# zraorg/ZRA

Measured on AMD Instinct MI355X. Metric: compress + RA-decompress GiB/s, 16 GiB @ 64 KiB frames, 1/2/4/8 MI355X, higher is better.
Workload: dtype u8

## Files before the change

zra_amd/csrc/zra_decode.hip:

```cpp
#include "zra_dev.h"
#include "zra_kernels.h"

using namespace zra_dev;

namespace {

constexpr int DEC_THREADS = 64;
constexpr int BATCH = 64;
#ifndef ZRA_XWIN
#define ZRA_XWIN 4032
#endif
constexpr u32 XPRE = 64, XWIN = ZRA_XWIN;
constexpr u32 BLOCK_MAX = 128u << 10;

__constant__ u32 c_ll_base[36] = {0,1,2,3,4,5,6,7,8,9,10,11,12,13,14,15,16,18,20,22,24,28,32,40,48,64,128,256,512,1024,2048,4096,8192,16384,32768,65536};
__constant__ u8 c_ll_bits[36] = {0,0,0,0,0,0,0,0,0,0,0,0,0,0,0,0,1,1,1,1,2,2,3,3,4,6,7,8,9,10,11,12,13,14,15,16};
__constant__ u32 c_ml_base[53] = {3,4,5,6,7,8,9,10,11,12,13,14,15,16,17,18,19,20,21,22,23,24,25,26,27,28,29,30,31,32,33,34,
                                  35,37,39,41,43,47,51,59,67,83,99,131,259,515,1027,2051,4099,8195,16387,32771,65539};
__constant__ u8 c_ml_bits[53] = {0,0,0,0,0,0,0,0,0,0,0,0,0,0,0,0,0,0,0,0,0,0,0,0,0,0,0,0,0,0,0,0,
                                 1,1,1,1,2,2,3,3,4,4,5,7,8,9,10,11,12,13,14,15,16};
__constant__ short c_ll_defnorm[36] = {4,3,2,2,2,2,2,2,2,2,2,2,2,1,1,1,2,2,2,2,2,2,2,2,2,3,2,1,1,1,1,1,-1,-1,-1,-1};
__constant__ short c_ml_defnorm[53] = {1,4,3,2,2,2,2,2,2,1,1,1,1,1,1,1,1,1,1,1,1,1,1,1,1,1,1,1,1,1,1,1,
                                       1,1,1,1,1,1,1,1,1,1,1,1,1,1,-1,-1,-1,-1,-1,-1,-1};
__constant__ short c_of_defnorm[29] = {1,1,1,1,1,1,2,2,2,1,1,1,1,1,1,1,1,1,1,1,1,1,1,1,-1,-1,-1,-1,-1};
__constant__ u16 c_huf_t0[16][2] = {{0,0},{0,0},{38,130},{448,128},{556,128},{714,128},{883,128},{897,128},{926,128},{947,128},{1107,128},{1177,128},{1242,128},{1349,128},{1455,128},{722,128}};
__constant__ u16 c_huf_t1[16][2] = {{1,1},{1,1},{1313,74},{1353,74},{1353,74},{1418,74},{1437,74},{1515,75},{1613,75},{1729,77},{2083,81},{2379,87},{2415,93},{2644,106},{2422,124},{1891,145}};

__device__ __forceinline__ u64 mk_seqsym(u32 baseValue, u32 addBits, u32 nbBits, u32 nextBase) {
  return (u64)baseValue | ((u64)addBits << 32) | ((u64)nbBits << 40) | ((u64)nextBase << 48);
}
__device__ __forceinline__ u32 mk_cell(u32 sym, u32 addBits, u32 nbBits, u32 nextBase) {
  return sym | (addBits << 8) | (nbBits << 16) | (nextBase << 20);
}

// ... 693 lines not shown
      {
        const u32 at = bpos + S.seqPos;
        const u32 got = stage(S.w1, at);
        (void)got;
        wsync();
      }
      const u8* const sw = S.w1 - S.seqPos;
      const u8* const swLim = S.w1 + STAGE_BYTES + 8;
      if (lane == 0) {
        parse_seq_header(S, sw + S.seqPos, bsize - S.seqPos);
        if (S.err) { S.lateErr = S.err; S.err = 0; S.nbSeq = 0; S.seqTables = 0; }
        if (S.alloc && S.nbSeq) {
          const u64 take = ((u64)S.nbSeq + 3) & ~3ull;
          const u64 at = atomicAdd((unsigned long long*)&a.counters[ZRA_DC_SEQCUR], (unsigned long long)take);
          if (at + take > a.seqCap) S.alloc = 0;
          S.seqBase = at;
        }
      }
      wsync();
      if (ALL && (!S.alloc || nBlk >= a.bpf)) { bail = true; break; }
      if (!S.alloc) {
        if (lane == 0) {
          save_persistent(S.hdrPos, produced0, hv0, hmb0, hns0, hx20);
          if (!FUSED) a.nextActive[atomicAdd(&a.counters[ZRA_DC_NNEXT], 1u)] = j;
        }
        handed = true; outcome = 2;
        wsync();
        break;
      }

      PPROF(10)
      const u32 nbSeq = S.nbSeq, regen = S.litRegen;
      const size_t jb = ALL ? (size_t)j * a.bpf + nBlk : (size_t)j;
      u32* const T = ALL ? a.blkTables + jb * ZRA_DEC_TBL_WORDS : a.tables + (size_t)j * ZRA_DEC_TBL_WORDS;
      if (S.seqTables) {
        for (int kind = 0; kind < 3; kind++) {
          const int k = kind == 0 ? 0 : kind == 1 ? 2 : 1;
          const u32 mode = k == 0 ? (S.seqModes >> 6) : k == 2 ? ((S.seqModes >> 4) & 3) : ((S.seqModes >> 2) & 3);
          if (lane == 0) {
            u32 tl = 0, ms = 0, used = 0;
            seq_table_parse(S, k, mode, sw + S.seqPos, bsize - S.seqPos, &tl, &ms, &used, swLim);
            S.seqPos += used; S.tl = tl; S.ms = ms;
            if (mode == 3) { u32 v = k == 0 ? S.llValid : k == 1 ? S.mlValid : S.ofValid; if (!v) S.err = ZE_CORRUPTION; }
            if (S.err) { S.lateErr = S.err; S.err = 0; }
          }
          wsync();
          PPROF(11)
          if (S.lateErr) break;
          const u32 tl = S.tl, ms = S.ms;
          u32* const G = T + (k == 0 ? ZRA_DEC_TBL_LL : k == 1 ? ZRA_DEC_TBL_ML : ZRA_DEC_TBL_OF);
          if (mode == 1) {
            if (lane == 0) {
              if (k == 2) { G[0] = mk_cell(ms, ms, 0, 0); S.ofShare = (ms > 22) ? 256u : 0u; }
              else G[0] = mk_cell(ms, k == 0 ? c_ll_bits[ms] : c_ml_bits[ms], 0, 0);
              if (FUSED) { u32* const GL = ldsT + (k == 0 ? ZRA_LDS_TBL_LL : k == 1 ? ZRA_LDS_TBL_ML : ZRA_LDS_TBL_OF); GL[0] = G[0]; if (k != 2) GL[1] = k == 0 ? c_ll_base[ms] : c_ml_base[ms]; }
            }
          } else if (mode != 3) {
            build_fse_dtable(S.stage, S.norm, ms, tl, k, S.spread, (u64*)S.w0, S.wnext, lane);
            wsync();
            const u32 words = (k == 2 ? 1u : 2u) << tl;
            if (!FUSED) for (u32 i = lane; i < (1u << tl); i += DEC_THREADS) G[i] = S.stage[k == 2 ? i : 2 * i];
            if (FUSED) { u32* const GL = ldsT + (k == 0 ? ZRA_LDS_TBL_LL : k == 1 ? ZRA_LDS_TBL_ML : ZRA_LDS_TBL_OF); for (u32 i = lane; i < words; i += DEC_THREADS) GL[i] = S.stage[i]; }
            if (k == 2) {
              u32 cnt = 0;
              for (u32 i = lane; i < (1u << tl); i += DEC_THREADS) cnt += (S.stage[i] & 0xFF) > 22;
              cnt = wave_sum(cnt);
              if (lane == 0) S.ofShare = cnt << (8 - tl);
            }
            wsync();
          }
          if (lane == 0 && mode != 3) {
            if (k == 0) { S.llLog = tl; S.llValid = 1; } else if (k == 1) { S.mlLog = tl; S.mlValid = 1; } else { S.ofLog = tl; S.ofValid = 1; }
          }
          if (ALL) {
            if (mode == 3 && prevT[k] && prevT[k] != G) {
              const u32 lg = k == 0 ? S.llLog : k == 1 ? S.mlLog : S.ofLog;
              for (u32 i = lane; i < (1u << lg); i += DEC_THREADS) G[i] = prevT[k][i];
            }
            prevT[k] = G;
          }
          wsync();
          PPROF(12)
        }
      }

      if (ALL) {
        ZraDecFrame* const D = &a.blkRecs[jb];
        if (lane == 0) {
          save_persistent_to(D, S.hdrPos, produced0, S.hufValid, S.hufMaxBits, S.hufNSym, S.hufX2);
          if (nBlk) { D->rep[0] = ZRA_REP_MARK(0); D->rep[1] = ZRA_REP_MARK(1); D->rep[2] = ZRA_REP_MARK(2); }
          D->bpos = bpos; D->bsize = bsize; D->blast = S.blkLast;
          D->litKind = S.litKind; D->litRegen = regen; D->litArg = S.litArg; D->litBase = S.litBase;
          D->litStreams = S.litStreams;
          for (int k = 0; k < 4; k++) { D->streamOff[k] = S.streamOff[k]; D->streamLen[k] = S.streamLen[k]; }
          D->hufErr = 0; D->lateErr = S.lateErr;
          D->nbSeq = S.lateErr ? 0u : nbSeq; D->seqPos = S.seqPos; D->seqBase = S.seqBase;
          D->longMode = 0;
          D->chainErr = 0; D->nSeqValid = 0; D->seqOut = 0; D->seqLit = 0; D->truncated = 0;
          a.pending[atomicAdd(&a.counters[ZRA_DC_NPENDING], 1u)] = (u32)jb;
          if (S.litKind == 2) a.hufJobs[atomicAdd(&a.counters[ZRA_DC_NHUF], 1u)] = (u32)jb;
          S.produced = produced0 + (S.blkLast ? 0u : ZRA_FMB_BLOCK); S.blkPos = bpos + bsize; S.frameEnd = S.blkLast;
          S.winLen = 0;
        }
        if (S.litKind == 2) {
          for (u32 i = lane; i < 256; i += DEC_THREADS) { D->weights[i] = S.weights[i]; D->hufStart[i] = S.hufStart[i]; }
        }
        if (S.lateErr) bail = true;
        nBlk++;
        wsync();
        continue;
// ... 381 lines not shown
    bc += nb; return v;
  }
  __device__ __forceinline__ u32 read_fast(u32 nb) {
    const u32 v = (u32)((c << (bc & 63)) >> ((64 - nb) & 63));
    bc += nb; return v;
  }
  __device__ __forceinline__ int reload() {
    if (bc > 64) return OVERFLOW;
    if (ptr >= 8) { ptr -= bc >> 3; bc &= 7; c = fetch(ptr); return UNFINISHED; }
    if (ptr == 0) return bc < 64 ? ENDOFBUFFER : COMPLETED;
    u32 nbBytes = bc >> 3; int r = UNFINISHED;
    if (ptr < nbBytes) { nbBytes = ptr; r = ENDOFBUFFER; }
    ptr -= nbBytes; bc -= nbBytes * 8; c = fetch(ptr);
    return r;
  }
  __device__ __forceinline__ void reload_quiet(bool wide, const u8* pad) {
    const u32 nb = bc <= 64 ? min(bc >> 3, ptr) : 0u;
    ptr -= nb; bc -= nb * 8;
    const u64 v = RING ? fetch(ptr) : ld64(wide ? base + ptr : pad);
    c = nb ? v : c;
  }
};
typedef ZdsT<false> Zds;

}

namespace {
template <bool LDSTAB>
__device__ __forceinline__ void chain_body(const ZraDecodeArgs& a, u32* const ldsTabs, u32* const baseLL, u32* const baseML, u32* const ldsRings = nullptr) {
  const int lane = threadIdx.x;
  const u32 nPend = a.counters[ZRA_DC_NPENDING];
  bool have = false, drained = false;
  ZraDecFrame* F = nullptr;
  const u32* T = nullptr;
  u64* sq = nullptr;
  ZdsT<LDSTAB> br; br.c = 0; br.bc = 0; br.ptr = 0; br.base = nullptr; br.ring = nullptr; br.rLo = 0;
  br.lim = a.body + a.bodySize; br.pf = make_uint4(0, 0, 0, 0); br.pfState = 0; br.pfAge = 0;
  if (LDSTAB) br.ring = (u8*)(ldsRings + (u32)lane * CHAIN_RING_WORDS);
  u32 sLL = 0, sOF = 0, sML = 0, rep0 = 1, rep1 = 4, rep2 = 8;
  u32 i = 0, nbSeq = 0, outPos = 0, litPos = 0, outCap = 0, regen = 0, produced0 = 0, limit = 0;
  u32 longMode = 0, err = 0, jErr = 0xFFFFFFFFu, valid = 0, validOut = 0, validLit = 0, truncated = 0;
  u64 q0 = 0, q1 = 0, q2 = 0;
  u32 eL = 0, eM = 0, eO = 0;
  bool wide = false; const u8* pad = nullptr;
  bool fresh = false; u32 freshJob = 0;
  const u16* const cells16 = (const u16*)ldsTabs + (size_t)lane * ZRA_DEC_TBL_WORDS;
  u32 logLL = 0, logML = 0, logOF = 0;
  auto fetch_cells = [&]() {
    if (LDSTAB) { eL = cells16[ZRA_DEC_TBL_LL + sLL]; eM = cells16[ZRA_DEC_TBL_ML + sML]; eO = cells16[ZRA_DEC_TBL_OF + sOF]; }
    else { eL = T[ZRA_DEC_TBL_LL + sLL]; eM = T[ZRA_DEC_TBL_ML + sML]; eO = T[ZRA_DEC_TBL_OF + sOF]; }
  };
  auto c_code = [&](u32 e) -> u32 { return e & 63u; };
  auto c_sbits = [&](u32 e, u32 lg) -> u32 { if (LDSTAB) return lg - (31u - (u32)__builtin_clz(e >> 6)); return (e >> 16) & 0xF; };
  auto c_sbase = [&](u32 e, u32 lg) -> u32 {
    if (LDSTAB) { const u32 v = e >> 6, hb = 31u - (u32)__builtin_clz(v); return (v ^ (1u << hb)) << (lg - hb); }
    return e >> 20;
  };
  baseLL[lane] = lane < 36 ? c_ll_base[lane] | (LDSTAB ? (u32)c_ll_bits[lane] << 24 : 0u) : 0u;
  baseML[lane] = lane < 53 ? c_ml_base[lane] | (LDSTAB ? (u32)c_ml_bits[lane] << 24 : 0u) : 0u;
  wsync();
  if (LDSTAB && (u32)lane >= ZRA_CHAIN_LDS_FRAMES) drained = true;

  auto finish = [&]() {
    { const u32 r = valid & 3u, b = valid - r;
      if (r >= 1) sq[b] = q0;
      if (r >= 2) sq[b + 1] = q1;
      if (r >= 3) sq[b + 2] = q2; }
    if (!err && !truncated) {
      if (regen - litPos > outCap - outPos) err = ZE_DSTSIZE_TOOSMALL;
    }
    F->chainErr = err; F->nSeqValid = valid; F->seqOut = validOut; F->seqLit = validLit; F->truncated = truncated;
    F->repOut[0] = rep0; F->repOut[1] = rep1; F->repOut[2] = rep2;
    have = false;
  };

  for (;;) {
    const u64 want = __ballot(!have && !drained);
    if (want) {
      u32 base = 0;
      const u32 cnt = (u32)__builtin_popcountll(want);
      if (lane == (int)__builtin_ctzll(want)) base = atomicAdd(&a.counters[ZRA_DC_QCHAIN], cnt);
      base = bcast_u32(base, (u32)__builtin_ctzll(want));
      if (!have && !drained) {
        const u32 idx = base + (u32)__builtin_popcountll(want & ((1ull << lane) - 1ull));
        if (idx >= nPend) drained = true;
        else {
          const u32 j = a.pending[idx];
          const size_t gj = frame_of(a, j);
          F = &a.frames[j];
          T = a.tables + (size_t)j * ZRA_DEC_TBL_WORDS;
          const u8* const blk = a.body + a.frameOff[gj * a.offStride] + F->bpos;
          nbSeq = F->nbSeq; regen = F->litRegen; produced0 = F->produced; longMode = F->longMode;
          outCap = a.outCap[gj] - produced0;
          limit = a.limit ? a.limit[gj] : 0xFFFFFFFFu;
          sq = a.seqs + F->seqBase;
          rep0 = F->rep[0]; rep1 = F->rep[1]; rep2 = F->rep[2];
          i = 0; outPos = 0; litPos = 0; err = 0; jErr = 0xFFFFFFFFu; valid = 0; validOut = 0; validLit = 0; truncated = 0;
          have = true; br.rLo = 0; br.pfState = 0;
          if (F->hufErr) { err = ZE_CORRUPTION; nbSeq = 0; finish(); }
          else if (F->lateErr) { err = F->lateErr; nbSeq = 0; finish(); }
          else if (nbSeq) {
            if (!br.init(blk + F->seqPos, F->bsize - F->seqPos)) { err = ZE_CORRUPTION; finish(); }
            else {
              logLL = F->llLog; logOF = F->ofLog; logML = F->mlLog;
              sLL = br.read(logLL); br.reload();
              sOF = br.read(logOF); br.reload();
              sML = br.read(logML); br.reload();
              wide = F->bsize - F->seqPos >= 8;
              pad = a.body + a.frameOff[gj * a.offStride];
              if (LDSTAB) { fresh = true; freshJob = j; } else fetch_cells();
            }
          }
        }
      }
    }
    if (LDSTAB) {
      u64 nm = __ballot(fresh);
      while (nm) {
        const u32 l = (u32)__builtin_ctzll(nm); nm &= nm - 1;
        const u32 jj = bcast_u32(freshJob, l);
        const uint4* const g4 = (const uint4*)(a.tables + (size_t)jj * ZRA_DEC_TBL_WORDS);
        uint2* const d2 = (uint2*)((u16*)ldsTabs + (size_t)l * ZRA_DEC_TBL_WORDS);
        const ZraDecFrame* const Fj = &a.frames[jj];
        const u32 lgL = Fj->llLog, lgM = Fj->mlLog, lgO = Fj->ofLog;
        for (u32 i = (u32)lane; i < ZRA_DEC_TBL_WORDS / 4; i += DEC_THREADS) {
          const uint4 q = g4[i];
          const u32 lg = 4 * i < ZRA_DEC_TBL_ML ? lgL : 4 * i < ZRA_DEC_TBL_OF ? lgM : lgO;
          auto pk = [&](u32 x) -> u32 { const u32 nb = min((x >> 16) & 0xFu, lg); return (x & 63u) | (((1u << (lg - nb)) | ((x >> 20) >> nb)) << 6); };
          d2[i] = make_uint2(pk(q.x) | (pk(q.y) << 16), pk(q.z) | (pk(q.w) << 16));
        }
      }
      if (__ballot(fresh)) wsync();
      if (fresh) { fetch_cells(); fresh = false; }
    }
    if (!__ballot(have)) break;

    if (have) {
      bool go = true;
      if (LDSTAB) { br.ring_guard(); br.ring_advance(); }
      if (i >= nbSeq) {
        if (!err && nbSeq && !longMode && br.reload() < Zds::COMPLETED) err = ZE_CORRUPTION;
        finish(); go = false;
      } else if (longMode) {
        if (br.reload() > Zds::COMPLETED) {
          if (jErr == 0xFFFFFFFFu || i <= jErr + 4) err = ZE_CORRUPTION;
          finish(); go = false;
        } else if (jErr != 0xFFFFFFFFu && i > jErr + 4) { finish(); go = false; }
      }
      if (go) {
        u32 ll = baseLL[c_code(eL)], ml = baseML[c_code(eM)], off;
        const u32 ofBits = LDSTAB ? c_code(eO) : (eO >> 8) & 0xFF, mlBits = LDSTAB ? ml >> 24 : (eM >> 8) & 0xFF, llBits = LDSTAB ? ll >> 24 : (eL >> 8) & 0xFF;
        if (LDSTAB) { ll &= 0xFFFFFFu; ml &= 0xFFFFFFu; }
        bool badOff = false;
        if (ofBits > 1) {
          off = ((1u << ofBits) - 3u) + br.read_fast(ofBits);
          if (a.bpf > 1 && off >= ZRA_REP_MARK_LO) badOff = true;
          rep2 = rep1; rep1 = rep0; rep0 = off;
        } else {
          const u32 ll0 = (ll == 0);
          if (ofBits == 0) {
            if (!ll0) off = rep0;
            else { off = rep1; rep1 = rep0; rep0 = off; }
          } else {
            const u32 idx = 1 + ll0 + br.read_fast(1);
            u32 t = idx == 3 ? rep0 - 1 : idx == 1 ? rep1 : rep2;
            t += !t;
            if (idx != 1) rep2 = rep1;
            rep1 = rep0; rep0 = off = t;
          }
        }
        if (mlBits) ml += br.read_fast(mlBits);
        if (llBits + mlBits + ofBits >= 57 - (9 + 9 + 8)) br.reload();
        if (llBits) ll += br.read_fast(llBits);
        sLL = c_sbase(eL, logLL) + br.read(c_sbits(eL, logLL));
        sML = c_sbase(eM, logML) + br.read(c_sbits(eM, logML));
        sOF = c_sbase(eO, logOF) + br.read(c_sbits(eO, logOF));
        fetch_cells();
        if (!longMode) br.reload_quiet(wide, pad);
        if (jErr == 0xFFFFFFFFu) {
          u32 e = 0;
          if (ll + ml > outCap - outPos) e = ZE_DSTSIZE_TOOSMALL;
          else if (ll > regen - litPos) e = ZE_CORRUPTION;
          else if (badOff || (off > produced0 + outPos + ll && !(a.bpf > 1 && off >= ZRA_REP_MARK_LO))) e = ZE_CORRUPTION;
          if (e) { jErr = i; err = e; if (!longMode) finish(); }
          else {
            const u64 qv = (u64)ll | ((u64)ml << 18) | ((u64)min(off, 0x0FFFFFFFu) << 36);
            const u32 slot = i & 3u;
            if (slot == 0) q0 = qv; else if (slot == 1) q1 = qv; else if (slot == 2) q2 = qv;
            else { uint4* d4 = (uint4*)(sq + (i - 3)); d4[0] = make_uint4((u32)q0, (u32)(q0 >> 32), (u32)q1, (u32)(q1 >> 32)); d4[1] = make_uint4((u32)q2, (u32)(q2 >> 32), (u32)qv, (u32)(qv >> 32)); }
            outPos += ll + ml; litPos += ll;
            valid = i + 1; validOut = outPos; validLit = litPos;
            if (produced0 + outPos >= limit) { truncated = 1; finish(); }
          }
        }
        i++;
      }
    }
  }
}
}

extern "C" __global__ void __launch_bounds__(DEC_THREADS)
zra_dec_chain_kernel(ZraDecodeArgs a) {
  __shared__ u32 baseLL[64], baseML[64];
  chain_body<false>(a, nullptr, baseLL, baseML);
}
extern "C" __global__ void __launch_bounds__(DEC_THREADS)
zra_dec_chain_lds_kernel(ZraDecodeArgs a) {
  extern __shared__ u32 chainLds[];
  chain_body<true>(a, chainLds + 128, chainLds, chainLds + 64, chainLds + 128 + ZRA_CHAIN_LDS_FRAMES * (ZRA_DEC_TBL_WORDS / 2));
}

namespace {
struct __attribute__((aligned(16))) ExecShared {
  union {
    u8 slot[BATCH][64];
    u8 win[XPRE + XWIN];
  };
  u32 endAt[BATCH];
  u32 matchAt[BATCH];
  u32 job;
};
}

#ifdef ZRA_DEC_PROFILE
__device__ unsigned long long zra_dec_prof[16];
#define XCNT(k, v) { if (lane == 0) atomicAdd(&zra_dec_prof[k], (unsigned long long)(v)); }
#define XTIME(k) { __builtin_amdgcn_s_waitcnt(0); const u64 n_ = __builtin_amdgcn_s_memtime(); if (lane == 0) atomicAdd(&zra_dec_prof[k], n_ - xpt_); xpt_ = n_; }
extern "C" __attribute__((visibility("default"))) void ZraHipDebugReadDecProfile(unsigned long long* out16, int reset) {
  (void)hipMemcpyFromSymbol(out16, HIP_SYMBOL(zra_dec_prof), sizeof(unsigned long long) * 16);
  if (reset) { unsigned long long z[16] = {0}; (void)hipMemcpyToSymbol(HIP_SYMBOL(zra_dec_prof), z, sizeof(z)); }
}
#else
#define XCNT(k, v)
#define XTIME(k)
#endif

namespace {
struct ExecCtx {
  u8* out; const u8* lit; u32 litKind; u8 rleByte;
  u32 outBase, litBase;
  const u8* src; u32 srcSize, produced0, regen;
  bool preValid;
// ... 632 lines not shown
```

zra_amd/csrc/zra_engine.hip:

```cpp
#include "zra_engine.h"
#include "zra_dev.h"
#include "zra_format.h"
#include "zra_env.h"
#include <algorithm>
#include <atomic>
#include <cstdio>
#include <chrono>
#include <cstdio>
#include <cstdlib>
#include <cstring>

extern "C" __global__ void zra_dec_parse_kernel(ZraDecodeArgs a);
extern "C" __global__ void zra_dec_huf_kernel(ZraDecodeArgs a);
extern "C" __global__ void zra_dec_chain_kernel(ZraDecodeArgs a);
extern "C" __global__ void zra_dec_chain_lds_kernel(ZraDecodeArgs a);
extern "C" __global__ void zra_dec_exec_kernel(ZraDecodeArgs a);
extern "C" __global__ void zra_dec_parse_all_kernel(ZraDecodeArgs a);
extern "C" __global__ void zra_dec_exec_all_kernel(ZraDecodeArgs a);
extern "C" __global__ void zra_ra_small_kernel(ZraDecodeArgs a, uint32_t* bail, const uint32_t* expect, uint32_t jobBase, unsigned long long* result);

using namespace zra_dev;

namespace zra_fmt {
uint32_t crc32(uint32_t crc, const void* data, size_t n) {
// ... 241 lines not shown
  if (stream_) (void)hipStreamSynchronize(stream_);
  for (DevBuf* b : {&raPlan_, &raLimit_, &raPieceBase_, &raPieces_, &decFrames_, &decTables_, &decLists_, &decCounters_, &decLits_, &decSeqs_, &roundN_, &status_, &produced_, &frameMeta_, &frameOff_, &outOff_, &expect_, &result_, &temp_, &qmeta_,
                    &encScan_, &hostIn_, &hostOut_, &seqScratch_, &mfFlags_, &decBlkRecs_, &decBlkTables_, &decBlkLists_})
    b->release();
  for (auto& x : encCtx_) for (DevBuf* b : {&x.tables, &x.seqs, &x.lits, &x.work, &x.slots, &x.misc, &x.ck, &x.sizes, &x.rec}) b->release();
  for (auto ev : evPool_) (void)hipEventDestroy(ev);
  for (auto ev : stageEv_) (void)hipEventDestroy(ev);
  if (stream2_) { (void)hipStreamSynchronize(stream2_); (void)hipStreamDestroy(stream2_); }
  for (auto st : pipeStreams_) if (st) { (void)hipStreamSynchronize(st); (void)hipStreamDestroy(st); }
  if (pinQ_) (void)hipHostFree(pinQ_);
  if (pinSmall_) (void)hipHostFree(pinSmall_);
  for (auto& ev : evR_) if (ev) (void)hipEventDestroy(ev);
  if (ev0_) (void)hipEventDestroy(ev0_);
  if (ev1_) (void)hipEventDestroy(ev1_);
  if (evWait_) (void)hipEventDestroy(evWait_);
  if (stream_) (void)hipStreamDestroy(stream_);
}

Status Engine::sync() { HIPCHK(hipSetDevice(device_)); HIPCHK(hipStreamSynchronize(stream_)); HIPCHK(hipStreamSynchronize(stream2_)); return ok(); }

Status Engine::wait_stream(hipStream_t producer) {
  HIPCHK(hipSetDevice(device_));
  HIPCHK(hipEventRecord(evWait_, producer));
  HIPCHK(hipStreamWaitEvent(stream_, evWait_, 0));
  HIPCHK(hipStreamWaitEvent(stream2_, evWait_, 0));
  return ok();
}

Status Engine::decode_scratch(ZraDecodeArgs& a, uint32_t maxFrameBytes) {
  const uint32_t n = a.nFrames;
  const uint64_t perFrame = std::min<uint64_t>((uint64_t)maxFrameBytes + 16, (128u << 10) + 16);
  const uint64_t litCap = std::max<uint64_t>((uint64_t)n * perFrame / 2, 1u << 20);
  const uint64_t seqCap = std::max<uint64_t>((uint64_t)n * perFrame * 3 / 32, 1u << 20);
  if (!decFrames_.reserve((size_t)n * sizeof(ZraDecFrame)) || !decTables_.reserve((size_t)n * ZRA_DEC_TBL_WORDS * 4) ||
      !decLists_.reserve((size_t)n * 16 + 64) || !decCounters_.reserve(ZRA_DC_WORDS * 4 + 64) || !decLits_.reserve(litCap + 64) ||
      !decSeqs_.reserve(seqCap * 8 + 64) || !status_.reserve((size_t)n * 4) || !produced_.reserve((size_t)n * 4) ||
      !frameMeta_.reserve((size_t)n * 8) || !result_.reserve(64))
    return zerr(64 );
  uint32_t* listA = decLists_.as<uint32_t>();
  a.pending = listA + 2 * (size_t)n; a.hufJobs = listA + 3 * (size_t)n;
  a.counters = decCounters_.as<uint32_t>();
  a.frames = decFrames_.as<ZraDecFrame>(); a.tables = decTables_.as<uint32_t>();
  a.lits = decLits_.as<uint8_t>(); a.litCap = litCap; a.seqs = decSeqs_.as<uint64_t>(); a.seqCap = seqCap;
  a.status = status_.as<uint32_t>(); a.produced = produced_.as<uint32_t>(); a.frameMeta = frameMeta_.as<uint32_t>();
  return ok();
}

Status Engine::decode_small(const ZraDecodeArgs& a0, const uint32_t* dExpect, uint32_t maxFrameBytes, uint32_t jobBase, unsigned long long* hResult, uint32_t* bailed) {
  ZraDecodeArgs a = a0;
  const uint32_t n = a.nFrames;
  const bool trace = ra_trace();
  auto t_last = std::chrono::steady_clock::now();
  auto mark = [&](const char* what) {
    if (!trace) return;
    const auto t = std::chrono::steady_clock::now();
    std::fprintf(stderr, "    small %-12s %7.1f us\n", what, std::chrono::duration<double, std::micro>(t - t_last).count());
    t_last = t;
  };
  { Status st = decode_scratch(a, maxFrameBytes); if (st.zra) return st; }
  mark("scratch");
  a.active = nullptr; a.nActive = n; a.round = 0; a.nextActive = decLists_.as<uint32_t>();
  if (!decCountersClean_) HIPCHK(hipMemsetAsync(a.counters, 0, ZRA_DC_WORDS * 4, stream_));
  decCountersClean_ = false;
  uint32_t* dBail = (uint32_t*)(result_.as<uint8_t>() + 8);
  HIPCHK(hipEventRecord(ev0_, stream_));
  hipLaunchKernelGGL(zra_ra_small_kernel, dim3(n), dim3(192), 0, stream_, a, dBail, dExpect, jobBase, result_.as<unsigned long long>());
  HIPCHK(hipEventRecord(ev1_, stream_));
  mark("launched");
  unsigned long long two[2] = {~0ull, ~0ull};
  HIPCHK(hipMemcpyAsync(two, result_.p, 16, hipMemcpyDeviceToHost, stream_));
  mark("queued rest");
  HIPCHK(hipStreamSynchronize(stream_));
  mark("sync");
  HIPCHK(hipGetLastError());
  if (hipMemsetAsync(a.counters, 0, ZRA_DC_WORDS * 4, stream_) == hipSuccess) decCountersClean_ = true;
  two[1] = 0xFFFFFFFFull - (two[1] & 0xFFFFFFFFull);
  *bailed = (uint32_t)two[1];
  if (!*bailed) *hResult = two[0];
  float ms = 0;
  if (hipEventElapsedTime(&ms, ev0_, ev1_) == hipSuccess) { lastKernelMs_ = ms; kstats_[4] += ms; kstats_[5] += 1; dstats_[5] += ms; dstats_[6] += 1; }
  return ok();
}

hipEvent_t Engine::stage_event() {
  if (stageEvNext_ == stageEv_.size()) { hipEvent_t e = nullptr; if (hipEventCreate(&e) != hipSuccess) return nullptr; stageEv_.push_back(e); }
  return stageEv_[stageEvNext_++];
}

Status Engine::decode_launch(const ZraDecodeArgs& a0, const uint32_t* dExpect, uint32_t maxFrameBytes, uint32_t jobBase, unsigned long long* hResult) {
  ZraDecodeArgs a = a0;
  const uint32_t n = a.nFrames;
  { Status st = decode_scratch(a, maxFrameBytes); if (st.zra) return st; }
  decCountersClean_ = false;
  uint32_t* listA = decLists_.as<uint32_t>(); uint32_t* listB = listA + n;
  if (!decOccParse_) {
    HIPCHK(hipOccupancyMaxActiveBlocksPerMultiprocessor(&decOccParse_, zra_dec_parse_kernel, 64, 0));
    HIPCHK(hipOccupancyMaxActiveBlocksPerMultiprocessor(&decOccExec_, zra_dec_exec_kernel, 64, 0));
    HIPCHK(hipOccupancyMaxActiveBlocksPerMultiprocessor(&decOccHuf_, zra_dec_huf_kernel, 64, 0));
    decOccParse_ = std::max(1, decOccParse_); decOccExec_ = std::max(1, decOccExec_); decOccHuf_ = std::max(1, decOccHuf_);
  }
  const int perCUParse = decOccParse_, perCUExec = decOccExec_;
  HIPCHK(hipEventRecord(ev0_, stream_));
  constexpr uint32_t chainWaves = 2;
  static const uint32_t chainLdsMin = (uint32_t)zra_env::env_int("ZRA_DEC_CHAIN_LDS_MIN", numCUs_ * 96);
  static const int chainLdsMode = zra_env::env_int("ZRA_DEC_CHAIN_LDS", 1);
  static const bool chainLdsOn = chainLdsMode != 0;
  constexpr uint32_t aheadCap = 16;
  if (!roundN_.reserve(4 * (aheadCap + 2) + 64)) return zerr(64);
  auto run_rounds = [&](ZraDecodeArgs& x, uint32_t nActive, const uint32_t* active, uint32_t round, uint32_t* lA, uint32_t* lB, uint32_t ahead) -> Status {
    uint32_t* const dN = roundN_.as<uint32_t>();
    while (nActive) {
      const uint32_t burst = std::max(1u, std::min(ahead, aheadCap));
      std::vector<hipEvent_t> evs;
      for (uint32_t bi = 0; bi < burst; bi++) {
        HIPCHK(hipMemsetAsync(x.counters, 0, ZRA_DC_WORDS * 4, stream_));
        x.active = active; x.nActive = nActive; x.round = round + bi;
        x.nActivePtr = bi ? dN + bi : nullptr;
        x.nextActive = (active == lA) ? lB : lA;
        const uint32_t gridParse = (uint32_t)std::min<uint64_t>(nActive, (uint64_t)numCUs_ * perCUParse);
        const uint32_t gridChain = (uint32_t)std::min<uint64_t>((nActive + 63) / 64, (uint64_t)numCUs_ * chainWaves);
        const uint32_t gridExec = (uint32_t)std::min<uint64_t>(nActive, (uint64_t)numCUs_ * perCUExec);
        hipEvent_t se[5];
        for (auto& e : se) { e = stage_event(); if (!e) return zerr(1); evs.push_back(e); }
        HIPCHK(hipEventRecord(se[0], stream_));
        hipLaunchKernelGGL(zra_dec_parse_kernel, dim3(gridParse), dim3(64), 0, stream_, x);
        HIPCHK(hipEventRecord(se[1], stream_));
        hipLaunchKernelGGL(zra_dec_huf_kernel, dim3((uint32_t)std::min<uint64_t>((nActive + ZRA_HUF_FRAMES - 1) / ZRA_HUF_FRAMES, (uint64_t)numCUs_ * decOccHuf_)), dim3(64), 0, stream_, x);
        HIPCHK(hipEventRecord(se[2], stream_));
        bool forked = false;
        if (chainLdsOn && nActive >= chainLdsMin) {
          if (!pipeStreams_[1]) { if (hipStreamCreateWithFlags(&pipeStreams_[1], hipStreamNonBlocking) != hipSuccess) { pipeStreams_[1] = nullptr; (void)hipGetLastError(); } }
          const size_t ldsBytes = (128 + (size_t)ZRA_CHAIN_LDS_FRAMES * (ZRA_DEC_TBL_WORDS / 2 + ZRA_CHAIN_RING_WORDS)) * 4;
          if (pipeStreams_[1] && !chainLdsAttr_) {
            if (hipFuncSetAttribute((const void*)zra_dec_chain_lds_kernel, hipFuncAttributeMaxDynamicSharedMemorySize, (int)ldsBytes) == hipSuccess) chainLdsAttr_ = 1;
            else { chainLdsAttr_ = -1; (void)hipGetLastError(); }
          }
          if (pipeStreams_[1] && chainLdsAttr_ > 0) {
            hipEvent_t eJoin = stage_event(); if (!eJoin) return zerr(1);
            HIPCHK(hipStreamWaitEvent(pipeStreams_[1], se[2], 0));
            hipLaunchKernelGGL(zra_dec_chain_lds_kernel, dim3((uint32_t)numCUs_), dim3(64), ldsBytes, pipeStreams_[1], x);
            HIPCHK(hipEventRecord(eJoin, pipeStreams_[1]));
            if (chainLdsMode != 2) hipLaunchKernelGGL(zra_dec_chain_kernel, dim3(gridChain), dim3(64), 0, stream_, x);
            HIPCHK(hipStreamWaitEvent(stream_, eJoin, 0));
            forked = true;
          }
        }
        if (!forked) hipLaunchKernelGGL(zra_dec_chain_kernel, dim3(gridChain), dim3(64), 0, stream_, x);
        HIPCHK(hipEventRecord(se[3], stream_));
        hipLaunchKernelGGL(zra_dec_exec_kernel, dim3(gridExec), dim3(64), 0, stream_, x);
        HIPCHK(hipEventRecord(se[4], stream_));
        HIPCHK(hipMemcpyAsync(dN + bi + 1, x.counters + ZRA_DC_NNEXT, 4, hipMemcpyDeviceToDevice, stream_));
        active = x.nextActive;
      }
      uint32_t next = 0;
      HIPCHK(hipMemcpyAsync(&next, dN + burst, 4, hipMemcpyDeviceToHost, stream_));
      HIPCHK(hipStreamSynchronize(stream_));
      HIPCHK(hipGetLastError());
      for (uint32_t bi = 0; bi < burst; bi++)
        for (int k = 0; k < 4; k++) { float m = 0; if (hipEventElapsedTime(&m, evs[5 * bi + k], evs[5 * bi + k + 1]) == hipSuccess) dstats_[k] += m; }
      dstats_[4] += burst;
      stageEvNext_ = 0;
      x.nActivePtr = nullptr;
      nActive = next; round += burst; ahead = 1;
      if (round > (1u << 20)) return zerr(1);
    }
    return ok();
  };
  static const int fmbEnv = zra_env::env_int("ZRA_DEC_FMB", 1);
  static const uint32_t fmbMin = (uint32_t)zra_env::env_int("ZRA_DEC_FMB_MIN", 64);
  const uint32_t bpf = (uint32_t)(((uint64_t)maxFrameBytes + ZRA_FMB_BLOCK - 1) / ZRA_FMB_BLOCK);
  bool fmb = fmbEnv != 0 && bpf >= 2 && maxFrameBytes <= (64u << 20) && n >= fmbMin && (uint64_t)n * bpf < (1ull << 30);
  uint32_t nRest = n;
  if (fmb) {
    const uint64_t nb = (uint64_t)n * bpf;
    const uint64_t litAll = std::max<uint64_t>((uint64_t)n * ((uint64_t)maxFrameBytes + 16) / 2, 1u << 20);
    const uint64_t seqAll = std::max<uint64_t>((uint64_t)n * ((uint64_t)maxFrameBytes + 16) * 3 / 32, 1u << 20);
    if (!decBlkRecs_.reserve((size_t)nb * sizeof(ZraDecFrame)) || !decBlkTables_.reserve((size_t)nb * ZRA_DEC_TBL_WORDS * 4) ||
        !decBlkLists_.reserve((size_t)(2 * nb + n) * 4 + 64) || !decLits_.reserve(litAll + 64) || !decSeqs_.reserve(seqAll * 8 + 64)) {
      (void)hipGetLastError();
      fmb = false;
    }
    a.lits = decLits_.as<uint8_t>(); a.seqs = decSeqs_.as<uint64_t>();
    if (fmb) {
      ZraDecodeArgs x = a;
      x.bpf = bpf; x.blkRecs = decBlkRecs_.as<ZraDecFrame>(); x.blkTables = decBlkTables_.as<uint32_t>();
      uint32_t* bl = decBlkLists_.as<uint32_t>();
      x.pending = bl; x.hufJobs = bl + nb; x.execList = bl + 2 * nb;
      x.litCap = litAll; x.seqCap = seqAll;
      x.active = nullptr; x.nActive = n; x.round = 0; x.nActivePtr = nullptr; x.nextActive = listA;
      HIPCHK(hipMemsetAsync(x.counters, 0, ZRA_DC_WORDS * 4, stream_));
      hipEvent_t se[5];
      for (auto& e : se) { e = stage_event(); if (!e) return zerr(1); }
      HIPCHK(hipEventRecord(se[0], stream_));
      hipLaunchKernelGGL(zra_dec_parse_all_kernel, dim3((uint32_t)std::min<uint64_t>(n, (uint64_t)numCUs_ * perCUParse)), dim3(64), 0, stream_, x);
      HIPCHK(hipEventRecord(se[1], stream_));
      ZraDecodeArgs y = x; y.frames = x.blkRecs; y.tables = x.blkTables;
      hipLaunchKernelGGL(zra_dec_huf_kernel, dim3((uint32_t)std::min<uint64_t>((nb + ZRA_HUF_FRAMES - 1) / ZRA_HUF_FRAMES, (uint64_t)numCUs_ * decOccHuf_)), dim3(64), 0, stream_, y);
      HIPCHK(hipEventRecord(se[2], stream_));
      const uint32_t gridChain = (uint32_t)std::min<uint64_t>((nb + 63) / 64, (uint64_t)numCUs_ * chainWaves);
      bool forked = false;
      if (chainLdsOn && nb >= chainLdsMin) {
        if (!pipeStreams_[1]) { if (hipStreamCreateWithFlags(&pipeStreams_[1], hipStreamNonBlocking) != hipSuccess) { pipeStreams_[1] = nullptr; (void)hipGetLastError(); } }
        const size_t ldsBytes = (128 + (size_t)ZRA_CHAIN_LDS_FRAMES * (ZRA_DEC_TBL_WORDS / 2 + ZRA_CHAIN_RING_WORDS)) * 4;
        if (pipeStreams_[1] && !chainLdsAttr_) {
          if (hipFuncSetAttribute((const void*)zra_dec_chain_lds_kernel, hipFuncAttributeMaxDynamicSharedMemorySize, (int)ldsBytes) == hipSuccess) chainLdsAttr_ = 1;
          else { chainLdsAttr_ = -1; (void)hipGetLastError(); }
        }
        if (pipeStreams_[1] && chainLdsAttr_ > 0) {
          hipEvent_t eJoin = stage_event(); if (!eJoin) return zerr(1);
          HIPCHK(hipStreamWaitEvent(pipeStreams_[1], se[2], 0));
          hipLaunchKernelGGL(zra_dec_chain_lds_kernel, dim3((uint32_t)numCUs_), dim3(64), ldsBytes, pipeStreams_[1], y);
          HIPCHK(hipEventRecord(eJoin, pipeStreams_[1]));
          if (chainLdsMode != 2) hipLaunchKernelGGL(zra_dec_chain_kernel, dim3(gridChain), dim3(64), 0, stream_, y);
          HIPCHK(hipStreamWaitEvent(stream_, eJoin, 0));
          forked = true;
        }
      }
      if (!forked) hipLaunchKernelGGL(zra_dec_chain_kernel, dim3(gridChain), dim3(64), 0, stream_, y);
      HIPCHK(hipEventRecord(se[3], stream_));
      hipLaunchKernelGGL(zra_dec_exec_all_kernel, dim3((uint32_t)std::min<uint64_t>(n, (uint64_t)numCUs_ * perCUExec)), dim3(64), 0, stream_, x);
      HIPCHK(hipEventRecord(se[4], stream_));
      uint32_t back = 0;
      HIPCHK(hipMemcpyAsync(&back, x.counters + ZRA_DC_NNEXT, 4, hipMemcpyDeviceToHost, stream_));
      HIPCHK(hipStreamSynchronize(stream_));
      HIPCHK(hipGetLastError());
      for (int k = 0; k < 4; k++) { float m = 0; if (hipEventElapsedTime(&m, se[k], se[k + 1]) == hipSuccess) dstats_[k] += m; }
      dstats_[4] += 1;
      stageEvNext_ = 0;
      nRest = back;
    }
  }
  Status st = fmb ? run_rounds(a, nRest, listA, 0, listA, listB, 1)
                  : run_rounds(a, n, nullptr, 0, listA, listB, (maxFrameBytes + (128u << 10) - 1) / (128u << 10));
  if (st.zra) return st;
  HIPCHK(hipEventRecord(ev1_, stream_));
  const uint32_t tb = 256;
// ... 296 lines not shown
```

zra_amd/csrc/zra_kernels.h:

```cpp
#pragma once
#include <stdint.h>
#include <stddef.h>

#ifndef ZRA_HUF_FRAMES
#define ZRA_HUF_FRAMES 2
#endif
#define ZRA_DEC_TBL_LL 0u
#define ZRA_DEC_TBL_ML 512u
#define ZRA_DEC_TBL_OF 1024u
#define ZRA_DEC_TBL_WORDS 1280u
#define ZRA_LDS_TBL_LL 0u
#define ZRA_LDS_TBL_ML 1024u
#define ZRA_LDS_TBL_OF 2048u
#define ZRA_LDS_TBL_WORDS 2304u
#define ZRA_CHAIN_LDS_FRAMES 59u
#define ZRA_CHAIN_RING_WORDS 36u

struct ZraDecFrame {
  uint32_t blkPos, produced, done;
  uint32_t hufValid, hufMaxBits, hufNSym, hufX2;
  uint32_t llValid, mlValid, ofValid, llLog, mlLog, ofLog, ofShare;
  uint32_t rep[3];
  uint32_t fcsLo, fcsHi, fcsHave, hasChecksum, bigWindow;
  uint32_t bpos, bsize, blast;
  uint32_t litKind, litRegen, litArg;
  uint32_t litStreams, streamOff[4], streamLen[4];
  uint32_t hufErr, lateErr;
  uint32_t nbSeq, seqPos, longMode;
  uint64_t litBase, seqBase;
  uint32_t chainErr, nSeqValid, seqOut, seqLit, truncated;
  uint32_t repOut[3];
  uint32_t nBlk, endPos, parseTrunc, pad1_;
  alignas(8) uint8_t weights[256];
  alignas(8) uint16_t hufStart[256];
};
#define ZRA_REP_MARK_LO 0x0C000000u
#define ZRA_REP_MARK(k) (ZRA_REP_MARK_LO + ((uint32_t)(k) << 24) + 0x00800000u)
#define ZRA_FMB_BLOCK (128u << 10)

struct ZraRaPiece { uint64_t dstOff; uint32_t srcOff, len; };

struct ZraDecodeArgs {
  const uint8_t* body;
  uint64_t bodySize;
  const uint64_t* frameOff;
  uint32_t offStride;
  uint8_t* out;
  const uint64_t* outOff;
  const uint32_t* outCap;
  uint32_t nFrames;
  const uint32_t* limit;
  const uint32_t* pieceBase;
  const ZraRaPiece* pieces;
  uint8_t* raOut;
  const uint32_t* active;
  uint32_t nActive;
  const uint32_t* nActivePtr;
  uint32_t round;
  uint32_t* counters;
  uint32_t* nextActive;
  uint32_t* pending;
  uint32_t* hufJobs;
  ZraDecFrame* frames;
  uint32_t* tables;
  uint8_t* lits; uint64_t litCap;
  uint64_t* seqs; uint64_t seqCap;
  uint32_t* status;
  uint32_t* produced;
  uint32_t* frameMeta;
  uint32_t debugSkip;
  uint32_t bpf;
  ZraDecFrame* blkRecs;
  uint32_t* blkTables;
  uint32_t* execList;
};
#define ZRA_DC_QPARSE 0
#define ZRA_DC_QCHAIN 1
#define ZRA_DC_QEXEC 2
#define ZRA_DC_NPENDING 3
#define ZRA_DC_NNEXT 4
#define ZRA_DC_NHUF 5
#define ZRA_DC_QHUF 10
#define ZRA_DC_LITCUR 6
#define ZRA_DC_SEQCUR 8
#define ZRA_DC_NEXEC 11
#define ZRA_DC_QEXECALL 12
#define ZRA_DC_WORDS 16

struct ZraEncParams {
  uint32_t windowLog, chainLog, hashLog, searchLog, minMatch, targetLength, strategy;
  uint32_t blockSize;
};

#define ZRA_OPT_NUM 4096u
struct ZraOptCell { int32_t price; uint32_t off, mlen, litlen, rep[3]; };
struct ZraOptMatch { uint32_t off, len; };
struct ZraOptState {
  uint32_t litFreq[256], litLengthFreq[36], matchLengthFreq[53], offCodeFreq[32];
  uint32_t litSum, litLengthSum, matchLengthSum, offCodeSum;
  uint32_t litSumBasePrice, litLengthSumBasePrice, matchLengthSumBasePrice, offCodeSumBasePrice;
  uint32_t predef, pad;
  ZraOptCell table[ZRA_OPT_NUM + 1];
  ZraOptMatch matches[ZRA_OPT_NUM + 1];
};

struct ZraFseCTable {
// ... 102 lines not shown
```

Before: 20.36.

## Store decode FSE tables as packed 16-bit cells in global memory

The parse stage now writes FSE decode tables to global memory as packed 16-bit cells (code plus a width/base encoding) instead of 32-bit stage words. The chain kernels read these cells directly, and the LDS chain variant copies a job's tables with plain 16-byte copies rather than repacking each entry on load. This halves table storage and global traffic and removes per-load conversion work. In exchange, the non-LDS path has to decode width and base with clz arithmetic on every symbol.

```diff
diff --git a/zra_amd/csrc/zra_cell.h b/zra_amd/csrc/zra_cell.h
--- /dev/null
+++ b/zra_amd/csrc/zra_cell.h
@@ -0,0 +1,22 @@
+#pragma once
+#include <stdint.h>
+
+#if defined(__HIPCC__) || defined(__CUDACC__)
+#define ZRA_CELL_FN __host__ __device__ __forceinline__
+#else
+#define ZRA_CELL_FN inline
+#endif
+
+ZRA_CELL_FN uint32_t zra_cell_pack(uint32_t code, uint32_t width, uint32_t base, uint32_t tableLog) {
+  return (code & 63u) | (((1u << (tableLog - width)) | (base >> width)) << 6);
+}
+ZRA_CELL_FN uint32_t zra_cell_from_stage(uint32_t x, uint32_t tableLog) {
+  const uint32_t w = (x >> 16) & 0xFu;
+  return zra_cell_pack(x, w < tableLog ? w : tableLog, x >> 20, tableLog);
+}
+ZRA_CELL_FN uint32_t zra_cell_code(uint32_t e) { return e & 63u; }
+ZRA_CELL_FN uint32_t zra_cell_width(uint32_t e, uint32_t tableLog) { return tableLog - (31u - (uint32_t)__builtin_clz(e >> 6)); }
+ZRA_CELL_FN uint32_t zra_cell_base(uint32_t e, uint32_t tableLog) {
+  const uint32_t v = e >> 6, hb = 31u - (uint32_t)__builtin_clz(v);
+  return (v ^ (1u << hb)) << (tableLog - hb);
+}
diff --git a/zra_amd/csrc/zra_decode.hip b/zra_amd/csrc/zra_decode.hip
--- a/zra_amd/csrc/zra_decode.hip
+++ b/zra_amd/csrc/zra_decode.hip
@@ -1,5 +1,6 @@
 #include "zra_dev.h"
 #include "zra_kernels.h"
+#include "zra_cell.h"
 
 using namespace zra_dev;
 
@@ -759,7 +760,7 @@
       PPROF(10)
       const u32 nbSeq = S.nbSeq, regen = S.litRegen;
       const size_t jb = ALL ? (size_t)j * a.bpf + nBlk : (size_t)j;
-      u32* const T = ALL ? a.blkTables + jb * ZRA_DEC_TBL_WORDS : a.tables + (size_t)j * ZRA_DEC_TBL_WORDS;
+      u16* const T = ALL ? a.blkTables + jb * ZRA_DEC_TBL_CELLS : a.tables + (size_t)j * ZRA_DEC_TBL_CELLS;
       if (S.seqTables) {
         for (int kind = 0; kind < 3; kind++) {
           const int k = kind == 0 ? 0 : kind == 1 ? 2 : 1;
@@ -775,18 +776,26 @@
           PPROF(11)
           if (S.lateErr) break;
           const u32 tl = S.tl, ms = S.ms;
-          u32* const G = T + (k == 0 ? ZRA_DEC_TBL_LL : k == 1 ? ZRA_DEC_TBL_ML : ZRA_DEC_TBL_OF);
+          u32* const G = (u32*)(T + (k == 0 ? ZRA_DEC_TBL_LL : k == 1 ? ZRA_DEC_TBL_ML : ZRA_DEC_TBL_OF));
           if (mode == 1) {
             if (lane == 0) {
-              if (k == 2) { G[0] = mk_cell(ms, ms, 0, 0); S.ofShare = (ms > 22) ? 256u : 0u; }
-              else G[0] = mk_cell(ms, k == 0 ? c_ll_bits[ms] : c_ml_bits[ms], 0, 0);
-              if (FUSED) { u32* const GL = ldsT + (k == 0 ? ZRA_LDS_TBL_LL : k == 1 ? ZRA_LDS_TBL_ML : ZRA_LDS_TBL_OF); GL[0] = G[0]; if (k != 2) GL[1] = k == 0 ? c_ll_base[ms] : c_ml_base[ms]; }
+              const u32 c = k == 2 ? mk_cell(ms, ms, 0, 0) : mk_cell(ms, k == 0 ? c_ll_bits[ms] : c_ml_bits[ms], 0, 0);
+              if (k == 2) S.ofShare = (ms > 22) ? 256u : 0u;
+              if (!FUSED) G[0] = zra_cell_from_stage(c, 0);
+              if (FUSED) { u32* const GL = ldsT + (k == 0 ? ZRA_LDS_TBL_LL : k == 1 ? ZRA_LDS_TBL_ML : ZRA_LDS_TBL_OF); GL[0] = c; if (k != 2) GL[1] = k == 0 ? c_ll_base[ms] : c_ml_base[ms]; }
             }
           } else if (mode != 3) {
             build_fse_dtable(S.stage, S.norm, ms, tl, k, S.spread, (u64*)S.w0, S.wnext, lane);
             wsync();
             const u32 words = (k == 2 ? 1u : 2u) << tl;
-            if (!FUSED) for (u32 i = lane; i < (1u << tl); i += DEC_THREADS) G[i] = S.stage[k == 2 ? i : 2 * i];
+            if (!FUSED) {
+              const u32 cells = 1u << tl, st = k == 2 ? 1u : 2u;
+              for (u32 i = lane; 2 * i < cells; i += DEC_THREADS) {
+                const u32 c0 = zra_cell_from_stage(S.stage[st * (2 * i)], tl);
+                const u32 c1 = 2 * i + 1 < cells ? zra_cell_from_stage(S.stage[st * (2 * i + 1)], tl) : 0u;
+                G[i] = c0 | (c1 << 16);
+              }
+            }
             if (FUSED) { u32* const GL = ldsT + (k == 0 ? ZRA_LDS_TBL_LL : k == 1 ? ZRA_LDS_TBL_ML : ZRA_LDS_TBL_OF); for (u32 i = lane; i < words; i += DEC_THREADS) GL[i] = S.stage[i]; }
             if (k == 2) {
               u32 cnt = 0;
@@ -802,7 +811,7 @@
           if (ALL) {
             if (mode == 3 && prevT[k] && prevT[k] != G) {
               const u32 lg = k == 0 ? S.llLog : k == 1 ? S.mlLog : S.ofLog;
-              for (u32 i = lane; i < (1u << lg); i += DEC_THREADS) G[i] = prevT[k][i];
+              for (u32 i = lane; 2 * i < (1u << lg); i += DEC_THREADS) G[i] = prevT[k][i];
             }
             prevT[k] = G;
           }
@@ -1250,7 +1259,7 @@
   const u32 nPend = a.counters[ZRA_DC_NPENDING];
   bool have = false, drained = false;
   ZraDecFrame* F = nullptr;
-  const u32* T = nullptr;
+  const u16* T = nullptr;
   u64* sq = nullptr;
   ZdsT<LDSTAB> br; br.c = 0; br.bc = 0; br.ptr = 0; br.base = nullptr; br.ring = nullptr; br.rLo = 0;
   br.lim = a.body + a.bodySize; br.pf = make_uint4(0, 0, 0, 0); br.pfState = 0; br.pfAge = 0;
@@ -1262,20 +1271,17 @@
   u32 eL = 0, eM = 0, eO = 0;
   bool wide = false; const u8* pad = nullptr;
   bool fresh = false; u32 freshJob = 0;
-  const u16* const cells16 = (const u16*)ldsTabs + (size_t)lane * ZRA_DEC_TBL_WORDS;
+  const u16* const ldsCells = (const u16*)ldsTabs + (size_t)lane * ZRA_DEC_TBL_CELLS;
   u32 logLL = 0, logML = 0, logOF = 0;
   auto fetch_cells = [&]() {
-    if (LDSTAB) { eL = cells16[ZRA_DEC_TBL_LL + sLL]; eM = cells16[ZRA_DEC_TBL_ML + sML]; eO = cells16[ZRA_DEC_TBL_OF + sOF]; }
+    if (LDSTAB) { eL = ldsCells[ZRA_DEC_TBL_LL + sLL]; eM = ldsCells[ZRA_DEC_TBL_ML + sML]; eO = ldsCells[ZRA_DEC_TBL_OF + sOF]; }
     else { eL = T[ZRA_DEC_TBL_LL + sLL]; eM = T[ZRA_DEC_TBL_ML + sML]; eO = T[ZRA_DEC_TBL_OF + sOF]; }
   };
-  auto c_code = [&](u32 e) -> u32 { return e & 63u; };
-  auto c_sbits = [&](u32 e, u32 lg) -> u32 { if (LDSTAB) return lg - (31u - (u32)__builtin_clz(e >> 6)); return (e >> 16) & 0xF; };
-  auto c_sbase = [&](u32 e, u32 lg) -> u32 {
-    if (LDSTAB) { const u32 v = e >> 6, hb = 31u - (u32)__builtin_clz(v); return (v ^ (1u << hb)) << (lg - hb); }
-    return e >> 20;
-  };
-  baseLL[lane] = lane < 36 ? c_ll_base[lane] | (LDSTAB ? (u32)c_ll_bits[lane] << 24 : 0u) : 0u;
-  baseML[lane] = lane < 53 ? c_ml_base[lane] | (LDSTAB ? (u32)c_ml_bits[lane] << 24 : 0u) : 0u;
+  auto c_code = [&](u32 e) -> u32 { return zra_cell_code(e); };
+  auto c_sbits = [&](u32 e, u32 lg) -> u32 { return zra_cell_width(e, lg); };
+  auto c_sbase = [&](u32 e, u32 lg) -> u32 { return zra_cell_base(e, lg); };
+  baseLL[lane] = lane < 36 ? c_ll_base[lane] | ((u32)c_ll_bits[lane] << 24) : 0u;
+  baseML[lane] = lane < 53 ? c_ml_base[lane] | ((u32)c_ml_bits[lane] << 24) : 0u;
   wsync();
   if (LDSTAB && (u32)lane >= ZRA_CHAIN_LDS_FRAMES) drained = true;
 
@@ -1306,7 +1312,7 @@
           const u32 j = a.pending[idx];
           const size_t gj = frame_of(a, j);
           F = &a.frames[j];
-          T = a.tables + (size_t)j * ZRA_DEC_TBL_WORDS;
+          T = a.tables + (size_t)j * ZRA_DEC_TBL_CELLS;
           const u8* const blk = a.body + a.frameOff[gj * a.offStride] + F->bpos;
           nbSeq = F->nbSeq; regen = F->litRegen; produced0 = F->produced; longMode = F->longMode;
           outCap = a.outCap[gj] - produced0;
@@ -1337,16 +1343,9 @@
       while (nm) {
         const u32 l = (u32)__builtin_ctzll(nm); nm &= nm - 1;
         const u32 jj = bcast_u32(freshJob, l);
-        const uint4* const g4 = (const uint4*)(a.tables + (size_t)jj * ZRA_DEC_TBL_WORDS);
-        uint2* const d2 = (uint2*)((u16*)ldsTabs + (size_t)l * ZRA_DEC_TBL_WORDS);
-        const ZraDecFrame* const Fj = &a.frames[jj];
-        const u32 lgL = Fj->llLog, lgM = Fj->mlLog, lgO = Fj->ofLog;
-        for (u32 i = (u32)lane; i < ZRA_DEC_TBL_WORDS / 4; i += DEC_THREADS) {
-          const uint4 q = g4[i];
-          const u32 lg = 4 * i < ZRA_DEC_TBL_ML ? lgL : 4 * i < ZRA_DEC_TBL_OF ? lgM : lgO;
-          auto pk = [&](u32 x) -> u32 { const u32 nb = min((x >> 16) & 0xFu, lg); return (x & 63u) | (((1u << (lg - nb)) | ((x >> 20) >> nb)) << 6); };
-          d2[i] = make_uint2(pk(q.x) | (pk(q.y) << 16), pk(q.z) | (pk(q.w) << 16));
-        }
+        const uint4* const g4 = (const uint4*)(a.tables + (size_t)jj * ZRA_DEC_TBL_CELLS);
+        uint4* const d4 = (uint4*)((u16*)ldsTabs + (size_t)l * ZRA_DEC_TBL_CELLS);
+        for (u32 i = (u32)lane; i < ZRA_DEC_TBL_BYTES / 16; i += DEC_THREADS) d4[i] = g4[i];
       }
       if (__ballot(fresh)) wsync();
       if (fresh) { fetch_cells(); fresh = false; }
@@ -1367,8 +1366,8 @@
       }
       if (go) {
         u32 ll = baseLL[c_code(eL)], ml = baseML[c_code(eM)], off;
-        const u32 ofBits = LDSTAB ? c_code(eO) : (eO >> 8) & 0xFF, mlBits = LDSTAB ? ml >> 24 : (eM >> 8) & 0xFF, llBits = LDSTAB ? ll >> 24 : (eL >> 8) & 0xFF;
-        if (LDSTAB) { ll &= 0xFFFFFFu; ml &= 0xFFFFFFu; }
+        const u32 ofBits = c_code(eO), mlBits = ml >> 24, llBits = ll >> 24;
+        ll &= 0xFFFFFFu; ml &= 0xFFFFFFu;
         bool badOff = false;
         if (ofBits > 1) {
           off = ((1u << ofBits) - 3u) + br.read_fast(ofBits);
@@ -1425,8 +1424,8 @@
 }
 extern "C" __global__ void __launch_bounds__(DEC_THREADS)
 zra_dec_chain_lds_kernel(ZraDecodeArgs a) {
-  extern __shared__ u32 chainLds[];
-  chain_body<true>(a, chainLds + 128, chainLds, chainLds + 64, chainLds + 128 + ZRA_CHAIN_LDS_FRAMES * (ZRA_DEC_TBL_WORDS / 2));
+  extern __shared__ __attribute__((aligned(16))) u32 chainLds[];
+  chain_body<true>(a, chainLds + 128, chainLds, chainLds + 64, chainLds + 128 + ZRA_CHAIN_LDS_FRAMES * (ZRA_DEC_TBL_BYTES / 4));
 }
 
 namespace {
diff --git a/zra_amd/csrc/zra_engine.hip b/zra_amd/csrc/zra_engine.hip
--- a/zra_amd/csrc/zra_engine.hip
+++ b/zra_amd/csrc/zra_engine.hip
@@ -297,7 +297,7 @@
   const uint64_t perFrame = std::min<uint64_t>((uint64_t)maxFrameBytes + 16, (128u << 10) + 16);
   const uint64_t litCap = std::max<uint64_t>((uint64_t)n * perFrame / 2, 1u << 20);
   const uint64_t seqCap = std::max<uint64_t>((uint64_t)n * perFrame * 3 / 32, 1u << 20);
-  if (!decFrames_.reserve((size_t)n * sizeof(ZraDecFrame)) || !decTables_.reserve((size_t)n * ZRA_DEC_TBL_WORDS * 4) ||
+  if (!decFrames_.reserve((size_t)n * sizeof(ZraDecFrame)) || !decTables_.reserve((size_t)n * ZRA_DEC_TBL_BYTES) ||
       !decLists_.reserve((size_t)n * 16 + 64) || !decCounters_.reserve(ZRA_DC_WORDS * 4 + 64) || !decLits_.reserve(litCap + 64) ||
       !decSeqs_.reserve(seqCap * 8 + 64) || !status_.reserve((size_t)n * 4) || !produced_.reserve((size_t)n * 4) ||
       !frameMeta_.reserve((size_t)n * 8) || !result_.reserve(64))
@@ -305,7 +305,7 @@
   uint32_t* listA = decLists_.as<uint32_t>();
   a.pending = listA + 2 * (size_t)n; a.hufJobs = listA + 3 * (size_t)n;
   a.counters = decCounters_.as<uint32_t>();
-  a.frames = decFrames_.as<ZraDecFrame>(); a.tables = decTables_.as<uint32_t>();
+  a.frames = decFrames_.as<ZraDecFrame>(); a.tables = decTables_.as<uint16_t>();
   a.lits = decLits_.as<uint8_t>(); a.litCap = litCap; a.seqs = decSeqs_.as<uint64_t>(); a.seqCap = seqCap;
   a.status = status_.as<uint32_t>(); a.produced = produced_.as<uint32_t>(); a.frameMeta = frameMeta_.as<uint32_t>();
   return ok();
@@ -366,7 +366,7 @@
   }
   const int perCUParse = decOccParse_, perCUExec = decOccExec_;
   HIPCHK(hipEventRecord(ev0_, stream_));
-  constexpr uint32_t chainWaves = 2;
+  constexpr uint32_t chainWaves = ZRA_CHAIN_WAVES;
   static const uint32_t chainLdsMin = (uint32_t)zra_env::env_int("ZRA_DEC_CHAIN_LDS_MIN", numCUs_ * 96);
   static const int chainLdsMode = zra_env::env_int("ZRA_DEC_CHAIN_LDS", 1);
   static const bool chainLdsOn = chainLdsMode != 0;
@@ -395,7 +395,7 @@
         bool forked = false;
         if (chainLdsOn && nActive >= chainLdsMin) {
           if (!pipeStreams_[1]) { if (hipStreamCreateWithFlags(&pipeStreams_[1], hipStreamNonBlocking) != hipSuccess) { pipeStreams_[1] = nullptr; (void)hipGetLastError(); } }
-          const size_t ldsBytes = (128 + (size_t)ZRA_CHAIN_LDS_FRAMES * (ZRA_DEC_TBL_WORDS / 2 + ZRA_CHAIN_RING_WORDS)) * 4;
+          const size_t ldsBytes = ZRA_CHAIN_LDS_BYTES;
           if (pipeStreams_[1] && !chainLdsAttr_) {
             if (hipFuncSetAttribute((const void*)zra_dec_chain_lds_kernel, hipFuncAttributeMaxDynamicSharedMemorySize, (int)ldsBytes) == hipSuccess) chainLdsAttr_ = 1;
             else { chainLdsAttr_ = -1; (void)hipGetLastError(); }
@@ -440,7 +440,7 @@
     const uint64_t nb = (uint64_t)n * bpf;
     const uint64_t litAll = std::max<uint64_t>((uint64_t)n * ((uint64_t)maxFrameBytes + 16) / 2, 1u << 20);
     const uint64_t seqAll = std::max<uint64_t>((uint64_t)n * ((uint64_t)maxFrameBytes + 16) * 3 / 32, 1u << 20);
-    if (!decBlkRecs_.reserve((size_t)nb * sizeof(ZraDecFrame)) || !decBlkTables_.reserve((size_t)nb * ZRA_DEC_TBL_WORDS * 4) ||
+    if (!decBlkRecs_.reserve((size_t)nb * sizeof(ZraDecFrame)) || !decBlkTables_.reserve((size_t)nb * ZRA_DEC_TBL_BYTES) ||
         !decBlkLists_.reserve((size_t)(2 * nb + n) * 4 + 64) || !decLits_.reserve(litAll + 64) || !decSeqs_.reserve(seqAll * 8 + 64)) {
       (void)hipGetLastError();
       fmb = false;
@@ -448,7 +448,7 @@
     a.lits = decLits_.as<uint8_t>(); a.seqs = decSeqs_.as<uint64_t>();
     if (fmb) {
       ZraDecodeArgs x = a;
-      x.bpf = bpf; x.blkRecs = decBlkRecs_.as<ZraDecFrame>(); x.blkTables = decBlkTables_.as<uint32_t>();
+      x.bpf = bpf; x.blkRecs = decBlkRecs_.as<ZraDecFrame>(); x.blkTables = decBlkTables_.as<uint16_t>();
       uint32_t* bl = decBlkLists_.as<uint32_t>();
       x.pending = bl; x.hufJobs = bl + nb; x.execList = bl + 2 * nb;
       x.litCap = litAll; x.seqCap = seqAll;
@@ -466,7 +466,7 @@
       bool forked = false;
       if (chainLdsOn && nb >= chainLdsMin) {
         if (!pipeStreams_[1]) { if (hipStreamCreateWithFlags(&pipeStreams_[1], hipStreamNonBlocking) != hipSuccess) { pipeStreams_[1] = nullptr; (void)hipGetLastError(); } }
-        const size_t ldsBytes = (128 + (size_t)ZRA_CHAIN_LDS_FRAMES * (ZRA_DEC_TBL_WORDS / 2 + ZRA_CHAIN_RING_WORDS)) * 4;
+        const size_t ldsBytes = ZRA_CHAIN_LDS_BYTES;
         if (pipeStreams_[1] && !chainLdsAttr_) {
           if (hipFuncSetAttribute((const void*)zra_dec_chain_lds_kernel, hipFuncAttributeMaxDynamicSharedMemorySize, (int)ldsBytes) == hipSuccess) chainLdsAttr_ = 1;
           else { chainLdsAttr_ = -1; (void)hipGetLastError(); }
diff --git a/zra_amd/csrc/zra_kernels.h b/zra_amd/csrc/zra_kernels.h
--- a/zra_amd/csrc/zra_kernels.h
+++ b/zra_amd/csrc/zra_kernels.h
@@ -8,13 +8,23 @@
 #define ZRA_DEC_TBL_LL 0u
 #define ZRA_DEC_TBL_ML 512u
 #define ZRA_DEC_TBL_OF 1024u
-#define ZRA_DEC_TBL_WORDS 1280u
+#define ZRA_DEC_TBL_CELLS 1280u
+#define ZRA_DEC_TBL_BYTES (ZRA_DEC_TBL_CELLS * 2u)
+static_assert(ZRA_DEC_TBL_BYTES % 16 == 0 && (ZRA_DEC_TBL_ML * 2) % 16 == 0 && (ZRA_DEC_TBL_OF * 2) % 16 == 0, "the chain kernels copy a job's tables as 16-byte pieces, the parse stage stores whole words");
 #define ZRA_LDS_TBL_LL 0u
 #define ZRA_LDS_TBL_ML 1024u
 #define ZRA_LDS_TBL_OF 2048u
 #define ZRA_LDS_TBL_WORDS 2304u
-#define ZRA_CHAIN_LDS_FRAMES 59u
+#ifndef ZRA_CHAIN_WAVES
+#define ZRA_CHAIN_WAVES 2u
+#endif
+#define ZRA_CHAIN_LDS_FRAMES_FIT ((((160u * 1024u - ZRA_CHAIN_WAVES * 1280u) / 1280u) * 1280u - 512u) / (ZRA_DEC_TBL_BYTES + 4u * 36u))
+#define ZRA_CHAIN_LDS_FRAMES (ZRA_CHAIN_LDS_FRAMES_FIT < 64u ? ZRA_CHAIN_LDS_FRAMES_FIT : 64u)
 #define ZRA_CHAIN_RING_WORDS 36u
+#define ZRA_CHAIN_LDS_BYTES ((128u + ZRA_CHAIN_LDS_FRAMES * (ZRA_DEC_TBL_BYTES / 4u + ZRA_CHAIN_RING_WORDS)) * 4u)
+static_assert(ZRA_CHAIN_RING_WORDS == 36u && ZRA_CHAIN_LDS_FRAMES <= 64 && (ZRA_CHAIN_LDS_BYTES + 1279u) / 1280u + ZRA_CHAIN_WAVES <= 128u,
+              "the LDS-table chain kernel's workgroup and the other chain kernel's waves must fit one CU's LDS together");
+static_assert(ZRA_CHAIN_WAVES != 2u || ZRA_CHAIN_LDS_FRAMES == 59u, "59 frames beside two waves");
 
 struct ZraDecFrame {
   uint32_t blkPos, produced, done;
@@ -62,7 +72,7 @@
   uint32_t* pending;
   uint32_t* hufJobs;
   ZraDecFrame* frames;
-  uint32_t* tables;
+  uint16_t* tables;
   uint8_t* lits; uint64_t litCap;
   uint64_t* seqs; uint64_t seqCap;
   uint32_t* status;
@@ -71,7 +81,7 @@
   uint32_t debugSkip;
   uint32_t bpf;
   ZraDecFrame* blkRecs;
-  uint32_t* blkTables;
+  uint16_t* blkTables;
   uint32_t* execList;
 };
 #define ZRA_DC_QPARSE 0
```

New measurement: 20.54, median of 6. Within noise of the previous version (+0.9%).
